# shuaigroup/Renormalizer

Hardware: AMD Instinct MI355X
Metric: TDVP-PS sweep site-updates/sec at (Nsite=50, Dbond=256, dphys=2/16) (higher is better)
Workload: dtype c128

## Files before the change

renormalizer_amd/csrc/mpse_gemm.hip:

```cpp
#include <cstdlib>

#include "mpse_device.h"
#include "mpse_internal.h"
#include "mpse_plans.h"

typedef double v4d __attribute__((ext_vector_type(4)));

static unsigned long long* gemm_trace_ptr(const mpse_ctx* ctx) {
  static const bool f0_only = [] {
    const char* e = getenv("MPSE_GEMM_TRACE_ONLY");
    return e && e[0] == 'f';
  }();
  return (ctx->prof_on && !f0_only) ? ctx->gemm_trace : nullptr;
}

namespace {

struct IdxMap {
  long long s_hi, s_lo;
  int ext, lo;
};

constexpr int GMAX_GRP = 8, GMAX_SEG = 4, GMAX_MIX = 8;
struct GMix {
  const double* src;
  int b, f, delta, pad;
};
struct GSeg {
  const double* A;
  const double* B;
  const unsigned char* am;
  const unsigned char* bm;
};
struct GGrp {
  GSeg seg[GMAX_SEG];
  double* C;
  int nseg;
  int use_beta;
};
struct GemmGroups {
  GGrp g[GMAX_GRP];
  int ngrp, tiles_m_grp, nkt_seg, am_pitch, bm_pitch;
  int split2, cpd;
  double* C2;
  const unsigned long long* flags;
  int nmix, mix_grp, mix_d, mix_wr;
  long long mix_ld;
  const double* mix_w;
  GMix mix[GMAX_MIX];
};

struct GemmArgs {
  const double* A;
  const double* B;
  double* C;
  IdxMap mA, kA, kB, nB, mC, nC;
  long long sbA, sbB, sbC;
  int M, N, K;
  int tiles_m, tiles_n;
  int mtiles_m, mtiles_n;
  int a_kfast, b_kfast;
  int conjA, conjB;
  int use_beta;
  double alpha_re, alpha_im, beta_re, beta_im;
  int skew;
  int die_group;
  int slice_fast;
  const int* perm;
  int ksplit;
  int kt_per_split;
  double* ws;
  const unsigned long long* amask;
  const unsigned long long* bmask;
  int nkw;
  unsigned long long* kt_counter;
  const int* skip;
  const double* dot_y;
  double* dot_part;
  const double* Cin;
  IdxMap mCin, nCin;
  unsigned long long* trace;
  GemmGroups gg;
};


__device__ __forceinline__ void dot_acc(double& re, double& im, double2 c, double2 y) {
  re += c.x * y.x + c.y * y.y;
  im += c.x * y.y - c.y * y.x;
}

__device__ __forceinline__ long long idx_off(const IdxMap& m, int i) {
  if (m.lo == 0x7fffffff) return (long long)i * m.s_lo;
  const int hi = i / m.lo;
  const int l = i - hi * m.lo;
  return (long long)hi * m.s_hi + (long long)l * m.s_lo;
}

#ifndef MPSE_GEMM_3M
#define MPSE_GEMM_3M 1
#endif
constexpr int BM = 64, BN = 64, BK = 16, LDK = BK + 1;

template <bool CA, bool CB, bool KS, int WS, int WI = 2, bool GRP = false>
__global__ __launch_bounds__(64 * WS * WS * (2 / WI), WS == 1 ? 1 : WI == 1 ? 4 : ((CA && CB) ? 2 : 3)) void k_gemm(const GemmArgs g) {
  static_assert(!GRP || (KS && WS == 2), "grouped launches use the single-level 64 x 64 kernel");
  constexpr int TBM = 32 * WS, TBN = 32 * WS, NT = 64 * WS * WS * (2 / WI);
  static_assert(WI == 2 || (WI == 1 && WS == 2), "eight-wave form only for 64 x 64 tiles");
  constexpr int LD = WS == 2 ? 80 : 48;
  constexpr int NLD = TBM * BK / NT;
  constexpr bool CC = CA || CB;
  constexpr int EA = CA ? 2 : 1, EB = CB ? 2 : 1, EC = CC ? 2 : 1;
  __shared__ double smem[(2 + (CA ? 1 : 0) + (CB ? 1 : 0)) * BK * LD];
  if (g.skip && *g.skip) return;
  const unsigned long long tr0 = g.trace ? __builtin_readcyclecounter() : 0ull;
  const unsigned long long rt0 = g.trace ? __builtin_amdgcn_s_memrealtime() : 0ull;
  unsigned long long tr1 = 0, tr2 = 0, tr3 = 0;
  double* sAr = smem;
  double* sAi = sAr + BK * LD;
  double* sBr = smem + (CA ? 2 : 1) * BK * LD;
  double* sBi = sBr + BK * LD;

  const int tid = threadIdx.x;
  const int lane = tid & 63;
  const int wave = tid >> 6;
  const int wm = WS == 2 ? wave >> 1 : 0, wn = WS == 2 ? wave & 1 : 0;
  constexpr int WROWS = 16 * WI;

  const int ntile = g.tiles_m * g.tiles_n;
  const int bid = blockIdx.x;
  int bs = bid / ntile;
  int t = bid - bs * ntile;
  int half = 0;
  if constexpr (GRP) {
    if (g.gg.split2) {
      if ((ntile & 7) == 0) {
        const int m2 = 2 * (ntile >> 3), r = bid >> 3, cpd = g.gg.cpd;
        const int q = (r < cpd || m2 <= cpd) ? r : (m2 - 1) - (r - cpd);
        half = q & 1;
        t = ((q >> 1) << 3) | (bid & 7);
      } else {
        half = bid & 1;
        t = bid >> 1;
      }
      bs = half;
    }
  }
  if (g.slice_fast) {
    t = bid / g.ksplit;
    bs = bid - t * g.ksplit;
  }
  const int b = bs / g.ksplit;
  const int ks_id = bs - b * g.ksplit;
  if (g.perm) t = g.perm[(ks_id & 1) ? ntile - 1 - t : t];
  int tm = t / g.tiles_n;
  int tn = t - tm * g.tiles_n;
  if (g.die_group == 1) {
    const int x = t & 7, j = t >> 3;
    tm = x + 8 * (j / g.tiles_n);
    tn = j % g.tiles_n;
  } else if (g.die_group == 2) {
    const int x = t & 7, j = t >> 3;
    tn = x + 8 * (j / g.tiles_m);
    tm = j % g.tiles_m;
  }
  if (g.skew && !g.perm && !g.die_group) tn = (tn + tm) % g.tiles_n;

  int grp = 0;
  if constexpr (GRP) {
    grp = tm / g.gg.tiles_m_grp;
    tm -= grp * g.gg.tiles_m_grp;
  }
  const GGrp& gp = g.gg.g[grp];
  const double* A = GRP ? gp.seg[0].A : g.A + (long long)b * g.sbA * EA;
  const double* B = GRP ? gp.seg[0].B : g.B + (long long)b * g.sbB * EB;
  double* C = GRP ? (half ? g.gg.C2 : gp.C) : g.C + (long long)b * g.sbC * EC;

  int ai[NLD], ak[NLD], bj[NLD], bk[NLD];
  long long aoff[NLD], boff[NLD];
#pragma unroll
  for (int r = 0; r < NLD; ++r) {
    if (g.a_kfast) {
      ak[r] = tid % BK;
      ai[r] = tid / BK + (NT / BK) * r;
    } else {
      ai[r] = tid % TBM;
      ak[r] = tid / TBM + (NT / TBM) * r;
    }
    if (g.b_kfast) {
      bk[r] = tid % BK;
      bj[r] = tid / BK + (NT / BK) * r;
    } else {
      bj[r] = tid % TBN;
      bk[r] = tid / TBN + (NT / TBN) * r;
    }
    int gi = min(tm * TBM + ai[r], g.M - 1);
    int gj = min(tn * TBN + bj[r], g.N - 1);
    aoff[r] = idx_off(g.mA, gi);
    boff[r] = idx_off(g.nB, gj);
  }

  double2 ra[NLD], rb[NLD];
  bool ka_in[NLD], kb_in[NLD];
  auto load_edge = [&](int kt) {
#pragma unroll
    for (int r = 0; r < NLD; ++r) {
      {
        const int k = kt * BK + ak[r];
        const bool kin = k < g.K;
        const int kc = kin ? k : g.K - 1;
        const long long ko = KS ? (long long)kc * g.kA.s_lo : idx_off(g.kA, kc);
        const double* p = A + (aoff[r] + ko) * EA;
        double2 v;
        if constexpr (CA) {
          v = *reinterpret_cast<const double2*>(p);
        } else {
          v.x = *p;
          v.y = 0.0;
        }
        ra[r] = v;
        ka_in[r] = kin;
      }
      {
        const int k = kt * BK + bk[r];
// ... 82 lines not shown
    const char* bt = b_col0 + (long long)kt * step_b;
    if constexpr (GRP) {
      const int q = kt / nkt_seg, l = kt - q * nkt_seg;
      at = seg_pick(seg_a, q) + (long long)l * step_a;
      bt = seg_pick(seg_b, q) + (long long)l * step_b;
    }
#pragma unroll
    for (int r = 0; r < NLD; ++r) {
      if constexpr (CA) {
        ra[r] = *reinterpret_cast<const double2*>(at + loa[r]);
      } else {
        ra[r].x = *reinterpret_cast<const double*>(at + loa[r]);
        ra[r].y = 0.0;
      }
      if constexpr (CB) {
        rb[r] = *reinterpret_cast<const double2*>(bt + lob[r]);
      } else {
        rb[r].x = *reinterpret_cast<const double*>(bt + lob[r]);
        rb[r].y = 0.0;
      }
    }
  };
  auto load_tile = [&](int kt) {
    if constexpr (GRP) {
      load_full(kt);
    } else if constexpr (KS) {
      if ((kt + 1) * BK <= g.K)
        load_full(kt);
      else
        load_ks(kt, false);
    } else {
      load_edge(kt);
    }
  };
  const double sgn_a = g.conjA ? -1.0 : 1.0, sgn_b = g.conjB ? -1.0 : 1.0;

  constexpr bool M3 = CA && CB && MPSE_GEMM_3M;
  v4d acc_re[WI][2], acc_im[WI][2], acc_t2[WI][2];
#pragma unroll
  for (int i = 0; i < WI; ++i)
#pragma unroll
    for (int j = 0; j < 2; ++j) {
      acc_re[i][j] = v4d{0, 0, 0, 0};
      acc_im[i][j] = v4d{0, 0, 0, 0};
      acc_t2[i][j] = v4d{0, 0, 0, 0};
    }

  constexpr int MASKW = 64;
  __shared__ unsigned long long s_mask[2][MASKW];
  const unsigned long long* am = nullptr;
  const unsigned long long* bm = nullptr;
  bool mlds = false;
  if constexpr (GRP) {
    if (g.nkw > 0 && g.nkw <= MASKW && g.gg.flags) {
      if (tid < g.nkw) {
        s_mask[0][tid] = g.gg.flags[((long long)(grp * g.gg.tiles_m_grp + tm) * g.tiles_n + tn) * g.nkw + tid];
        s_mask[1][tid] = 0x0101010101010101ull;
      }
      __syncthreads();
      mlds = true;
      am = s_mask[0];
    } else if (g.nkw > 0 && g.nkw <= MASKW) {
      unsigned char* f0 = reinterpret_cast<unsigned char*>(s_mask[0]);
      for (int t = tid; t < g.nkw * 8; t += NT) {
        unsigned char v = 0;
        if (t < nkt_all) {
          const int q = t / nkt_seg, l = t - q * nkt_seg;
          const GSeg& sg = gp.seg[q];
          v = 1;
          if (sg.am) v &= sg.am[(long long)tm * g.gg.am_pitch + l];
          if (sg.bm) v &= sg.bm[(long long)tn * g.gg.bm_pitch + l];
        }
        f0[t] = v;
      }
      if (tid < g.nkw) s_mask[1][tid] = 0x0101010101010101ull;
      __syncthreads();
      mlds = true;
      am = s_mask[0];
    }
    if (g.gg.split2) {
      if (mlds) {
        auto word_of = [&](int w) {
          unsigned long long x = s_mask[0][w] & 0x0101010101010101ull;
          const int valid = nkt_all - 8 * w;
          if (valid < 8) x &= valid > 0 ? (1ull << (8 * valid)) - 1ull : 0ull;
          return x;
        };
        int n = 0;
        for (int w = 0; w < g.nkw; ++w) n += __popcll(word_of(w));
        auto pos_of = [&](int i) {
          if (i >= n) return nkt_all;
          int seen = 0;
          for (int w = 0; w < g.nkw; ++w) {
            unsigned long long x = word_of(w);
            const int c = __popcll(x);
            if (seen + c > i) {
              for (int skip = i - seen; skip > 0; --skip) x &= x - 1;
              return (w << 3) + (__builtin_ctzll(x) >> 3);
            }
            seen += c;
          }
          return nkt_all;
        };
        kt_begin = half == 0 ? 0 : pos_of(n / 2);
        kt_end = half == 0 ? pos_of(n / 2) : nkt_all;
      } else {
        kt_begin = half == 0 ? 0 : nkt_all / 2;
        kt_end = half == 0 ? nkt_all / 2 : nkt_all;
      }
    }
  } else if constexpr (KS) {
    if (g.amask) am = g.amask + ((long long)b * g.mtiles_m + (tm * TBM) / BM) * g.nkw;
    if (g.bmask) bm = g.bmask + ((long long)b * g.mtiles_n + (tn * TBN) / BN) * g.nkw;
    if ((am || bm) && g.nkw <= MASKW) {
      if (tid < g.nkw) {
        s_mask[0][tid] = am ? am[tid] : 0x0101010101010101ull;
        s_mask[1][tid] = bm ? bm[tid] : 0x0101010101010101ull;
      }
      __syncthreads();
      mlds = true;
    }
  }
  auto next_kt = [&](int from) -> int {
    if (!am && !bm) return from;
    while (from < kt_end) {
      const int w = from >> 3;
      unsigned long long word = 0x0101010101010101ull;
      if (mlds) {
        word &= s_mask[0][w] & s_mask[1][w];
      } else {
        if (am) word &= am[w];
        if (bm) word &= bm[w];
      }
      word &= ~0ull << ((from & 7) * 8);
      if (word) {
        const int kt = (w << 3) + (__builtin_ctzll(word) >> 3);
        return kt < kt_end ? kt : kt_end;
      }
      from = (w + 1) << 3;
    }
    return kt_end;
  };
  int kt = next_kt(kt_begin);
  if (g.trace) tr1 = __builtin_readcyclecounter();
  if (kt < kt_end) {
    load_tile(kt);
  }
  const int frow = lane & 15, fk = lane >> 4;
  const int sai = g.a_kfast ? LDK : 1, sak = g.a_kfast ? 1 : LD;
  const int sbj = g.b_kfast ? LDK : 1, sbk = g.b_kfast ? 1 : LD;
  int wofa[NLD], wofb[NLD], rofa[WI], rofb[2];
#pragma unroll
  for (int r = 0; r < NLD; ++r) {
    wofa[r] = ai[r] * sai + ak[r] * sak;
    wofb[r] = bj[r] * sbj + bk[r] * sbk;
  }
#pragma unroll
  for (int i = 0; i < 2; ++i) {
// ... 362 lines not shown
        }
      }
    }
  }
  if constexpr (WS == 2) {
    if (g.dot_y) {
      __shared__ double s_dot[2 * (NT / 64)];
      dre = wave_sum(dre);
      dim = wave_sum(dim);
      if (lane == 0) {
        s_dot[2 * wave] = dre;
        s_dot[2 * wave + 1] = dim;
      }
      __syncthreads();
      dre = dim = 0.0;
#pragma unroll
      for (int w = 0; w < NT / 64; ++w) {
        dre += s_dot[2 * w];
        dim += s_dot[2 * w + 1];
      }
      if (tid == 0) {
        const long long slot = (long long)bs * ntile + (long long)tm * g.tiles_n + tn;
        g.dot_part[2 * slot] = dre;
        g.dot_part[2 * slot + 1] = dim;
      }
    }
  }
}

__device__ __forceinline__ void bitonic_desc(unsigned* key, int tid, int n) {
  for (int size = 2; size <= n; size <<= 1)
    for (int stride = size >> 1; stride > 0; stride >>= 1) {
      if (tid < (n >> 1)) {
        const int lo = 2 * tid - (tid & (stride - 1)), hi = lo + stride;
        const bool desc = (lo & size) == 0;
        const unsigned a = key[lo], b = key[hi];
        if ((a < b) == desc) {
          key[lo] = b;
          key[hi] = a;
        }
      }
      __syncthreads();
    }
}
__device__ __forceinline__ int pow2_at_least(int x) {
  int n = 2;
  while (n < x) n <<= 1;
  return n;
}
__global__ __launch_bounds__(1024) void k_tile_order(const unsigned long long* __restrict__ amask,
                                                       const unsigned long long* __restrict__ bmask, int nkw, int nkt,
                                                       int tiles_m, int tiles_n, int by_die, int* __restrict__ perm,
                                                       const int* __restrict__ skip, const GemmGroups gg,
                                                       unsigned char* __restrict__ flags_out, int flags_pitch) {
  if (skip && *skip) return;
  __shared__ unsigned key[2048], ckey[2048];
  __shared__ int colw[2048];
  __shared__ unsigned char die_of[2048];
  const int ntile = tiles_m * tiles_n, tid = threadIdx.x;
  const bool part = by_die && tiles_n % 8 == 0 && tiles_n <= 2048;
  for (int c = tid; c < 2048; c += 1024) colw[c] = 0;
  __syncthreads();
  for (int i = tid; i < 2048; i += 1024) {
    unsigned cnt = 0;
    if (i < ntile) {
      const int tm = i / tiles_n, tn = i - tm * tiles_n;
      if (gg.ngrp > 0) {
        const int grp = tm / gg.tiles_m_grp, tml = tm - grp * gg.tiles_m_grp;
        const GGrp& G = gg.g[grp];
        for (int q = 0; q < G.nseg; ++q)
          for (int l = 0; l < gg.nkt_seg; ++l) {
            unsigned v = 1;
            if (G.seg[q].am) v &= G.seg[q].am[(long long)tml * gg.am_pitch + l];
            if (G.seg[q].bm) v &= G.seg[q].bm[(long long)tn * gg.bm_pitch + l];
            cnt += v;
            if (flags_out) flags_out[(long long)i * flags_pitch + q * gg.nkt_seg + l] = (unsigned char)v;
          }
        if (flags_out)
          for (int l = G.nseg * gg.nkt_seg; l < flags_pitch; ++l) flags_out[(long long)i * flags_pitch + l] = 0;
      } else {
        for (int w = 0; w < nkw; ++w) {
          unsigned long long x = 0x0101010101010101ull;
          if (amask) x &= amask[(long long)tm * nkw + w];
          if (bmask) x &= bmask[(long long)tn * nkw + w];
          const int valid = nkt - 8 * w;
          if (valid < 8) x &= (1ull << (8 * valid)) - 1ull;
          cnt += __popcll(x);
        }
      }
      if (part) atomicAdd(&colw[tn], (int)cnt);
    }
    key[i] = cnt;
  }
  __syncthreads();
  if (part) {
    for (int c = tid; c < 2048; c += 1024) ckey[c] = c < tiles_n ? ((unsigned)colw[c] << 11) | (unsigned)(2047 - c) : 0u;
    __syncthreads();
    bitonic_desc(ckey, tid, pow2_at_least(tiles_n));
    for (int r = tid; r < tiles_n; r += 1024) {
      const int c = 2047 - (int)(ckey[r] & 2047u), r16 = r & 15;
      die_of[c] = (unsigned char)(r16 < 8 ? r16 : 15 - r16);
    }
    __syncthreads();
  }
  for (int i = tid; i < 2048; i += 1024) {
    unsigned k = 0;
    if (i < ntile) {
      const unsigned die = part ? die_of[i % tiles_n] : 0u;
      k = (die << 28) | (key[i] << 16) | (unsigned)(0xFFFF - i);
    }
    key[i] = k;
  }
  __syncthreads();
  bitonic_desc(key, tid, pow2_at_least(ntile));
  const int per_die = ntile / 8;
  for (int i = tid; i < ntile; i += 1024) {
    const int s = part ? (7 - (i & 7)) * per_die + (i >> 3) : i;
    perm[i] = 0xFFFF - (int)(key[s] & 0xFFFFu);
  }
}

template <bool CC>
__global__ __launch_bounds__(256) void k_splitk_reduce(const GemmArgs g, int batch) {
  constexpr int EC = CC ? 2 : 1;
  if (g.skip && *g.skip) return;
  const long long mn = (long long)g.M * g.N;
  const int rows = g.M * batch;
  double dre = 0.0, dim = 0.0;
  for (int row = blockIdx.y; row < rows; row += gridDim.y) {
    const int b = row / g.M;
    const int i = row - b * g.M;
    const double* wrow = g.ws + ((long long)b * g.ksplit * mn + (long long)i * g.N) * EC;
    double* crow = g.C + ((long long)b * g.sbC + idx_off(g.mC, i)) * EC;
    for (int j = blockIdx.x * 256 + threadIdx.x; j < g.N; j += gridDim.x * 256) {
      const double* w = wrow + (long long)j * EC;
      double xr = 0, xi = 0;
      int s = 0;
      for (; s + 4 <= g.ksplit; s += 4) {
        if constexpr (CC) {
          const double2 v0 = *reinterpret_cast<const double2*>(w + (long long)s * mn * EC);
          const double2 v1 = *reinterpret_cast<const double2*>(w + (long long)(s + 1) * mn * EC);
          const double2 v2 = *reinterpret_cast<const double2*>(w + (long long)(s + 2) * mn * EC);
          const double2 v3 = *reinterpret_cast<const double2*>(w + (long long)(s + 3) * mn * EC);
          xr += v0.x;
          xi += v0.y;
          xr += v1.x;
          xi += v1.y;
          xr += v2.x;
          xi += v2.y;
          xr += v3.x;
          xi += v3.y;
        } else {
          const double v0 = w[(long long)s * mn], v1 = w[(long long)(s + 1) * mn];
          const double v2 = w[(long long)(s + 2) * mn], v3 = w[(long long)(s + 3) * mn];
          xr += v0;
          xr += v1;
          xr += v2;
          xr += v3;
        }
      }
      for (; s < g.ksplit; ++s) {
        if constexpr (CC) {
          const double2 v = *reinterpret_cast<const double2*>(w + (long long)s * mn * EC);
          xr += v.x;
          xi += v.y;
        } else {
          xr += w[(long long)s * mn];
        }
      }
      const long long co = idx_off(g.nC, j);
      double* p = crow + co * EC;
// ... 332 lines not shown
  if (p.leave_slices) {
    g.ws = static_cast<double*>(rq->slices);
    rq->slices_used = g.ksplit;
  } else if (g.ksplit > 1) {
    MPSE_TRY(WSB.alloc(p.ws_bytes));
    g.ws = WSB.as<double>();
  }
  if (p.dot_producers) {
    g.dot_y = static_cast<const double*>(dot->y);
    g.dot_part = dot->part;
    dot->nb_out = (int)p.dot_producers;
  }
  mpse_ctx::ProfRec rec;
  const int variant = (ca ? 1 : 0) + (cb ? 2 : 0);
  const double mnk = double(g.M) * double(g.N) * double(g.K) * double(d->batch);
  const bool prof_this = prof_begin(
      ctx, variant, mnk * ((ca && cb) ? 8.0 : (ca || cb) ? 4.0 : 2.0),
      double(d->batch) * (double(g.M) * g.K * (ca ? 16 : 8) + double(g.K) * g.N * (cb ? 16 : 8) +
                          double(g.M) * g.N * ((ca || cb) ? 16 : 8) * (g.use_beta ? 2 : 1)),
      &rec);
  g.kt_counter = prof_this && ctx->prof_ktiles ? ctx->prof_ktiles + variant : nullptr;

  OccMask ma, mb;
  if (p.masks) {
    g.nkw = p.nkw;
    const bool sa = skip_zero & 1, sb = skip_zero & 2;
    const SolveScope::OccKey ka = occ_key(g.A, g.mA, g.kA, g.sbA, d->batch, ca);
    const SolveScope::OccKey kb = occ_key(g.B, g.nB, g.kB, g.sbB, d->batch, cb);
    SolveScope* const keep_a = sa && sc && sc->in_env(g.A) ? sc : nullptr;
    SolveScope* const keep_b = sb && sc && sc->in_env(g.B) ? sc : nullptr;
    const void* centre = (sb && sc && sc->in_krylov(g.B) && d->batch == 1 && (long long)occ_bytes(kb) == sc->cmask.bytes)
                             ? sc->cmask.ptr : nullptr;
    const size_t tmp_a = sa && !keep_a ? occ_bytes(ka) : 0, tmp_b = sb && !keep_b && !centre ? occ_bytes(kb) : 0;
    if (tmp_a + tmp_b) MPSE_TRY(MSK.alloc(tmp_a + tmp_b));
    if (sa) MPSE_TRY(occ_mask_source(ctx, keep_a, ka, nullptr, MSK.p, &ma));
    if (sb) MPSE_TRY(occ_mask_source(ctx, keep_b, kb, centre, MSK.as<char>() + tmp_a, &mb));
    if (ma.scan || mb.scan) {
      const OccOperand oa = occ_operand(ka, g.mA, g.kA, g.a_kfast, ma), ob = occ_operand(kb, g.nB, g.kB, g.b_kfast, mb);
      const dim3 og((p.nkt + 3) / 4, oa.tiles > ob.tiles ? oa.tiles : ob.tiles, (unsigned)(2 * d->batch));
      hipLaunchKernelGGL(k_tile_occ, og, dim3(256), 0, ctx->stream, oa, ob, g.K, g.nkw, (int)d->batch, g.skip);
    }
    g.amask = static_cast<const unsigned long long*>(ma.mask);
    g.bmask = static_cast<const unsigned long long*>(mb.mask);
  }

  if (p.order) {
    SolveScope* const keep = sc && sc->keeps_env_masks && ma.stable && mb.stable ? sc : nullptr;
    int* pp = nullptr;
    bool sort = false;
    MPSE_TRY(perm_source(ctx, keep, {g.amask, g.bmask, g.tiles_m, g.tiles_n, p.nkt, nullptr},
                         size_t(g.tiles_m) * g.tiles_n * sizeof(int), PERM, &pp, &sort));
    if (sort)
      hipLaunchKernelGGL(k_tile_order, dim3(1), dim3(1024), 0, ctx->stream, g.amask, g.bmask, g.nkw, p.nkt, g.tiles_m,
                         g.tiles_n, 1, pp, g.skip, GemmGroups(), (unsigned char*)nullptr, 0);
    g.perm = pp;
  }

  count_paths(ctx->gemm_paths, p, d->batch > 1);
  const bool reduce = g.ksplit > 1 && !p.leave_slices;
  launch_gemm(ctx, g, p.nwg, ca, cb, p.fast, p.wide, false, reduce ? dim3((unsigned)p.rgx, (unsigned)p.rgy) : dim3(0),
              (int)d->batch);
  if (prof_this) prof_end(ctx, rec);
  MPSE_HIP(ctx, hipGetLastError());
  return MPSE_OK;
}

int occ_mask_get(mpse_ctx* ctx, SolveScope* sc, const void* ptr, int dtype, mpse_index r, mpse_index k,
                 TmpBuf& tmp, const unsigned char** flags, int* pitch, bool* stable) {
  IdxMap rm, km;
  if (!to_map(r, &rm) || !to_map(k, &km) || !is_single(km))
    return mpse_fail(ctx, MPSE_ERR_SHAPE, "occupancy scan: K index must be single level");
  const SolveScope::OccKey key = occ_key(ptr, rm, km, 0, 1, dtype == MPSE_C128);
  SolveScope* const keep = sc && sc->in_env(ptr) ? sc : nullptr;
  OccMask m;
  if (!keep) MPSE_TRY(tmp.alloc(occ_bytes(key)));
  MPSE_TRY(occ_mask_source(ctx, keep, key, nullptr, tmp.p, &m));
  if (m.scan) {
    const OccOperand oa = occ_operand(key, rm, km, fastest(km) <= fastest(rm), m);
    OccOperand ob = oa;
    ob.tiles = 0;
    hipLaunchKernelGGL(k_tile_occ, dim3(((key.K + BK - 1) / BK + 3) / 4, key.tiles, 2), dim3(256), 0, ctx->stream, oa, ob,
                       key.K, key.nkw, 1, sc ? sc->skip : nullptr);
    MPSE_HIP(ctx, hipGetLastError());
  }
  *flags = static_cast<const unsigned char*>(m.mask);
  *pitch = key.nkw * 8;
  *stable = m.stable;
  return MPSE_OK;
}

static double mix_sources(const GroupedDesc& d) {
  int n = 0;
  for (int t = 0; t < d.nmix; ++t) {
    bool seen = false;
    for (int u = 0; u < t; ++u) seen = seen || d.mix[u].src == d.mix[t].src;
    n += seen ? 0 : 1;
  }
  return n > 1 ? double(n - 1) : 0.0;
}

int gemm_grouped(mpse_ctx* ctx, const GroupedDesc& d, SolveScope* sc, MatvecReq::Dot* dot) {
  GemmArgs g = {};
  if (d.ngrp < 1 || d.ngrp > GMAX_GRP) return mpse_fail(ctx, MPSE_ERR_ARG, "grouped product: 1 .. %d groups", GMAX_GRP);
  if (!fill_maps(g, d.ma, d.ka, d.kb, d.nb, d.mc, d.nc))
    return mpse_fail(ctx, MPSE_ERR_SHAPE, "grouped product: extent out of range");
  if (g.M != g.mC.ext || g.N != g.nC.ext || g.K != g.kB.ext) return mpse_fail(ctx, MPSE_ERR_SHAPE, "grouped product: extents disagree");
  if (g.M == 0 || g.N == 0) return MPSE_OK;
// ... 24 lines not shown
    gg.g[i].C = static_cast<double*>(s.C);
    gg.g[i].nseg = s.nseg;
    gg.g[i].use_beta = s.beta != 0.0 ? 1 : 0;
    if (s.beta != 0.0 && s.beta != 1.0) return mpse_fail(ctx, MPSE_ERR_ARG, "grouped product: beta must be 0 or 1");
    any_beta = any_beta || s.beta != 0.0;
    for (int q = 0; q < s.nseg; ++q) {
      if (!s.seg[q].A || !s.seg[q].B) return mpse_fail(ctx, MPSE_ERR_ARG, "grouped product: null operand");
      gg.g[i].seg[q] = GSeg{static_cast<const double*>(s.seg[q].A), static_cast<const double*>(s.seg[q].B), s.seg[q].am, s.seg[q].bm};
      any_mask = any_mask || s.seg[q].am || s.seg[q].bm;
    }
    max_seg = s.nseg > max_seg ? s.nseg : max_seg;
    segs += s.nseg;
  }
  g.A = gg.g[0].seg[0].A, g.B = gg.g[0].seg[0].B, g.C = gg.g[0].C;
  g.use_beta = any_beta;
  if (d.nmix > 0) {
    if (!ca || d.nmix > GMAX_MIX || d.mix_grp < 0 || d.mix_grp >= d.ngrp || d.grp[d.mix_grp].beta != 1.0 || !d.mix_w ||
        d.mix_d < 1 || BM % d.mix_d != 0 || g.M % BM != 0 || d.mix_wr < 1 || d.mix_ld < g.N)
      return mpse_fail(ctx, MPSE_ERR_ARG, "grouped product: bad epilogue mix");
    gg.nmix = d.nmix, gg.mix_grp = d.mix_grp, gg.mix_d = d.mix_d, gg.mix_wr = d.mix_wr, gg.mix_ld = d.mix_ld;
    gg.mix_w = static_cast<const double*>(d.mix_w);
    for (int t = 0; t < d.nmix; ++t) {
      if (!d.mix[t].src || d.mix[t].delta <= -d.mix_d || d.mix[t].delta >= d.mix_d)
        return mpse_fail(ctx, MPSE_ERR_ARG, "grouped product: bad epilogue mix term");
      gg.mix[t] = GMix{static_cast<const double*>(d.mix[t].src), d.mix[t].b, d.mix[t].f, d.mix[t].delta, 0};
    }
  }

  const int nkt_max = max_seg * gg.nkt_seg;
  const mpse_plan::GroupedPlan p = mpse_plan::grouped_plan(g.M, g.N, d.ngrp, nkt_max, any_mask, d.split2, ca, n_cu_of(ctx));
  const long long ntile = (long long)p.tiles_m * p.tiles_n;
  if (ntile > 0x7fffffffLL) return mpse_fail(ctx, MPSE_ERR_SHAPE, "grouped product: grid too large");
  g.tiles_m = p.tiles_m;
  g.nkw = p.nkw;
  g.die_group = p.die_group;
  if (dot && d.ngrp == 1 && p.nwg >= 1 && p.nwg <= dot->cap) {
    g.dot_y = static_cast<const double*>(dot->y);
    g.dot_part = dot->part;
    dot->nb_out = (int)p.nwg;
  }
  mpse_ctx::ProfRec rec;
  const int variant = (ca ? 1 : 0) + (cb ? 2 : 0);
  const double mnk = double(g.M) * double(g.N) * double(g.K) * segs;
  const bool prof_this = prof_begin(ctx, variant, mnk * ((ca && cb) ? 8.0 : 4.0),
                                    segs * (double(g.M) * g.K * (ca ? 16 : 8) + double(g.K) * g.N * 16.0) +
                                        double(d.ngrp) * double(g.M) * g.N * 16.0 * (any_beta ? 2 : 1) +
                                        mix_sources(d) * double(g.M) * g.N * 16.0,
                                    &rec);
  g.kt_counter = prof_this && ctx->prof_ktiles ? ctx->prof_ktiles + variant : nullptr;

  TmpBuf PERM(ctx);
  if (p.order) {
    const size_t perm_bytes = (size_t(ntile) * sizeof(int) + 7) & ~size_t(7), flag_pitch = size_t(g.nkw) * 8;
    int* pp = nullptr;
    bool sort = false;
    MPSE_TRY(perm_source(ctx, sc && sc->keeps_env_masks && d.masks_stable ? sc : nullptr,
                         {gg.g[0].seg[0].am, gg.g[0].seg[0].bm, g.tiles_m, g.tiles_n, nkt_max + 1000 * d.ngrp, nullptr},
                         perm_bytes + size_t(ntile) * flag_pitch, PERM, &pp, &sort));
    if (sort)
      hipLaunchKernelGGL(k_tile_order, dim3(1), dim3(1024), 0, ctx->stream, (const unsigned long long*)nullptr,
                         (const unsigned long long*)nullptr, 0, nkt_max, g.tiles_m, g.tiles_n, d.split2 ? 0 : 1, pp,
                         g.skip, gg, reinterpret_cast<unsigned char*>(pp) + perm_bytes, (int)flag_pitch);
    g.perm = pp;
    g.gg.flags = reinterpret_cast<const unsigned long long*>(reinterpret_cast<const char*>(pp) + perm_bytes);
  }

  count_paths(ctx->gemm_paths, d);
  launch_gemm(ctx, g, p.nwg, ca, cb, true, p.wide, true);
  if (prof_this) prof_end(ctx, rec);
  MPSE_HIP(ctx, hipGetLastError());
  return MPSE_OK;
}

extern "C" int mpse_gemm(mpse_ctx* ctx, const mpse_gemm_desc* d, const void* A, const void* B, void* C) {
  if (ctx && d && MPSE_RECORDING(ctx)) {
    const mpse_gemm_desc dc = *d;
    ctx->defer_ops[ctx->defer_recording].push_back([ctx, dc, A, B, C] { return mpse_gemm(ctx, &dc, A, B, C); });
    return MPSE_OK;
  }
  return gemm_impl(ctx, d, A, B, C, d ? (d->skip_zero_tiles & 3) : 0, nullptr, nullptr);
}

extern "C" int mpse_gemm_path_stats(mpse_ctx* ctx, int64_t* counts, int n) {
  if (!ctx || n < 0 || (n > 0 && !counts)) return MPSE_ERR_ARG;
  for (int i = 0; i < n && i < mpse_ctx::GP_COUNT; ++i) counts[i] = ctx->gemm_paths[i];
  return MPSE_OK;
}

int gemm_call(mpse_ctx* ctx, int dta, int dtb, int conja, int conjb, mpse_index ma, mpse_index ka, mpse_index kb,
              mpse_index nb, mpse_index mc, mpse_index nc, int64_t batch, int64_t sba, int64_t sbb, int64_t sbc,
              const void* A, const void* B, void* C, double alpha, double beta, int skip_zero, SolveScope* sc,
              ProductReq* rq) {
  mpse_gemm_desc d;
  d.dtype_a = dta;
  d.dtype_b = dtb;
  d.conj_a = conja;
  d.conj_b = conjb;
  d.m_a = ma;
  d.k_a = ka;
  d.k_b = kb;
  d.n_b = nb;
  d.m_c = mc;
  d.n_c = nc;
  d.batch = batch;
  d.sb_a = sba;
  d.sb_b = sbb;
  d.sb_c = sbc;
  d.alpha_re = alpha;
  d.alpha_im = 0.0;
  d.beta_re = beta;
  d.beta_im = 0.0;
  d.skip_zero_tiles = skip_zero;
  return gemm_impl(ctx, &d, A, B, C, skip_zero, sc, rq);
}

extern "C" int mpse_transpose_inner(mpse_ctx* ctx, int dtype, void* out, const void* in, int64_t d0, int64_t d1,
// ... 17 lines not shown
```

renormalizer_amd/csrc/mpse_internal.h:

```cpp
#pragma once
#include <hip/hip_runtime.h>

#include <cstdarg>
#include <cstdlib>
#include <cstdint>
#include <cstdio>
#include <cstring>
#include <functional>
#include <map>
#include <memory>
#include <mutex>
#include <string>
#include <unordered_map>
#include <vector>

#include "../../include/mpsengine.h"

struct mpse_ctx {
  int device = 0;
  hipStream_t stream = nullptr;
  int n_cu = 0;
  char err[512] = {0};
  char dev_name[128] = {0};

// ... 15 lines not shown
  std::vector<ProfRec> prof_pending;
  std::vector<hipEvent_t> prof_free_events;
  static constexpr int PROF_NVAR = 8;
  int64_t prof_svd_sweeps = 0;
  double prof_ms[PROF_NVAR] = {0};
  double prof_flops[PROF_NVAR] = {0};
  double prof_bytes[PROF_NVAR] = {0};
  int64_t prof_launches[PROF_NVAR] = {0};
  unsigned long long* prof_ktiles = nullptr;

  char* stage = nullptr;
  char* stage_dev = nullptr;
  size_t stage_size = 0, stage_pos = 0;

  enum PinnedSlot {
    PIN_SCALAR2 = 0,
    PIN_FLAG = 8,
    PIN_LZ_SCAL = 16,
    PIN_LZ_CTL = 24,
    PIN_ENV_UNIT = 32,
    PIN_PCG_CTL = 40,
    PIN_DAVIDSON = 64,
    PIN_BATCH_CTL = 3700,
    PIN_QR_STATUS = 3990,
    PIN_SLOTS_END = 4000,
    PIN_DOUBLES = 4096,
    PIN_SEQ = PIN_DOUBLES - 1
  };
  double* pinned = nullptr;
  double* pinned_dev = nullptr;
  unsigned long long publish_seq = 0;
  double* dscratch = nullptr;
  unsigned int flag_gen = 0;
  std::unordered_map<unsigned long long, int> lz_hint;
  struct WSiteEntry {
    std::shared_ptr<void> info;
    size_t bytes = 0;
  };
  std::unordered_map<const void*, WSiteEntry> wsite_info;
  std::vector<std::function<int()>> defer_ops[2];
  int defer_recording = -1;
  int defer_armed = -1;
  bool defer_hold = false;
  std::vector<void*> defer_frees;
  struct CMask {
    const void* ptr = nullptr;
    long long bytes = 0;
  } cmask_pending;
  unsigned long long* gemm_trace = nullptr;
  bool gemm_trace_checked = false;
  long long f0_launches[2] = {0, 0};
  enum GemmPath {
    GP_LAUNCH, GP_GENERAL, GP_WIDE, GP_SPLIT_B1, GP_SPLIT_BN, GP_DIE1, GP_DIE2, GP_SKEW, GP_ORDER, GP_MASK,
    GP_MASK_GLOBAL, GP_GROUPED, GP_GROUPED_SPLIT2, GP_GROUPED_MIX, GP_WMIX, GP_COUNT
  };
  long long gemm_paths[GP_COUNT] = {0};
  long long qr_chol_calls = 0, qr_chol_fallbacks = 0, qr_calls = 0;
  bool qr_optimistic = false;
  int qr_scheme = -1;
  int* qr_words_dev = nullptr;
  long long lz_batch_members = 0, lz_batch_single = 0;
  enum LzPath {
    LP_SYNC, LP_ASYNC_DONE, LP_HOST_FIRST, LP_HOST_LATER, LP_LIMIT, LP_BD_ASYNC, LP_BD_SYNC, LP_FULL, LP_CONV,
    LP_NOCONV, LP_MERGED, LP_WAITS, LP_GROW, LP_PARTS, LP_VMASK, LP_UNVEC, LP_RESCALE, LP_ALIAS_RESTART, LP_COUNT
  };
  long long lz_paths[LP_COUNT] = {0};
  enum PcgStat {
    PS_SOLVES, PS_ITERS, PS_MATVECS, PS_WAITS, PS_END_TOL, PS_END_MAXITER, PS_END_CURVATURE, PS_TWOLAYER, PS_MASKED,
    PS_COUNT
  };
  long long pcg_stats[PS_COUNT] = {0};
  enum PcgSumStat { PSS_SOLVES, PSS_ITERS, PSS_TERM_APPLIES, PSS_WAITS, PSS_DIAGS, PSS_COUNT };
  long long pcg_sum_stats[PSS_COUNT] = {0};
  enum PcgBatchStat { PB_MEMBERS, PB_SINGLE, PB_SETS, PB_MATVEC_LAUNCHES, PB_WAITS, PB_COUNT };
  long long pcg_batch_stats[PB_COUNT] = {0};
  enum OverlapStat { OV_CHAIN, OV_ENQUEUED, OV_SITES, OV_COUNT };
  long long overlap_stats[OV_COUNT] = {0};
  enum SandwichStat { SW_CHAIN, SW_ENQUEUED, SW_SITES, SW_COUNT };
  long long sandwich_stats[SW_COUNT] = {0};
  enum CorrStat { CR_CHAIN, CR_ENQUEUED, CR_SITES, CR_ENTRIES, CR_COUNT };
  long long corr_stats[CR_COUNT] = {0};
};
int qr_words(mpse_ctx* ctx);

int mpse_fail(mpse_ctx* ctx, int code, const char* fmt, ...);
inline int mpse_bind(mpse_ctx* ctx) {
  int cur = -1;
  if (hipGetDevice(&cur) == hipSuccess && cur == ctx->device) return MPSE_OK;
  if (hipSetDevice(ctx->device) != hipSuccess) return mpse_fail(ctx, MPSE_ERR_HIP, "hipSetDevice(%d) failed", ctx->device);
  return MPSE_OK;
}
int stage_h2d(mpse_ctx* ctx, void* dst, const void* src_host, size_t bytes);
int device_zero(mpse_ctx* ctx, void* dst, size_t bytes);
inline void wsite_written(mpse_ctx* ctx, const void* dst, size_t bytes) {
  if (!dst || !bytes) return;
  std::lock_guard<std::mutex> lock(ctx->pool_mu);
  if (ctx->wsite_info.empty()) return;
  const char* lo = static_cast<const char*>(dst);
  for (auto it = ctx->wsite_info.begin(); it != ctx->wsite_info.end();) {
    const char* w = static_cast<const char*>(it->first);
    if (lo < w + it->second.bytes && w < lo + bytes)
      it = ctx->wsite_info.erase(it);
    else
      ++it;
  }
}
void prof_drain(mpse_ctx* ctx);
// ... 294 lines not shown
```

renormalizer_amd/engine.py:

```python
import collections
import ctypes as C
import math
import os
import threading

import numpy as np

_HERE = os.path.dirname(os.path.abspath(__file__))
LIB_PATH = os.environ.get("RENO_MPSENGINE") or os.path.join(_HERE, "csrc", "libmpsengine.so")

F64, C128 = 0, 1
MPSE_OK, MPSE_ERR_OOM, MPSE_ERR_SHAPE, MPSE_ERR_NOCONV, MPSE_ERR_HIP, MPSE_ERR_ARG = 0, 1, 2, 3, 4, 5
DOMAIN_L, DOMAIN_R = 0, 1

STATUS = {0: "OK", 1: "OOM", 2: "SHAPE", 3: "NOCONV", 4: "HIP", 5: "ARG"}


PcgResult = collections.namedtuple("PcgResult", "status iters relres lvalue")


class EngineError(RuntimeError):
    pass


# ... 664 lines not shown
    @staticmethod
    def corr_dims(sites):
        rows = []
        for i, t in enumerate(sites):
            if t.ndim not in (3, 4):
                raise ValueError(f"mps_corr: site {i} has shape {t.shape}")
            rows.append([t.shape[0], t.shape[1], t.shape[2] if t.ndim == 4 else 1, t.shape[-1]])
        return rows

    def mps_corr(self, sites, sel, x_mats, y_mats, z_mats):
        rows = self.corr_dims(sites)
        n, nsel = len(rows), len(sel)
        if n == 0 or nsel == 0 or not (len(x_mats) == len(y_mats) == len(z_mats) == nsel):
            raise ValueError(f"mps_corr: {n} sites, {nsel} selected, {len(x_mats)}/{len(y_mats)}/{len(z_mats)} matrices")
        packed = []
        for mats in (x_mats, y_mats, z_mats):
            flat = []
            for k, m in zip(sel, mats):
                m = np.ascontiguousarray(m, dtype=np.complex128)
                d = rows[k][1] if 0 <= int(k) < n else m.shape[0]
                if m.shape != (d, d):
                    raise ValueError(f"mps_corr: a local matrix of site {k} has shape {m.shape}, the site has d = {d}")
                flat.append(m.reshape(-1))
            packed.append(np.ascontiguousarray(np.concatenate(flat)).view(np.float64))
        dims = (C.c_int64 * (4 * n))(*[int(x) for r in rows for x in r])
        out = np.zeros((nsel, nsel), dtype=np.complex128)
        self._check(self.lib.mpse_mps_corr(
            self.ctx, n, *_site_args(sites), dims, nsel, (C.c_int * nsel)(*[int(k) for k in sel]),
            *[p.ctypes.data_as(_dblp) for p in packed], out.ctypes.data_as(_dblp)))
        return out

    def block_qr_stats(self):
        a, b, c = C.c_int64(), C.c_int64(), C.c_int64()
        self._check(self.lib.mpse_block_qr_stats(self.ctx, C.byref(a), C.byref(b), C.byref(c)))
        return a.value, b.value, c.value

    def heff_fused_stats(self):
        a, b = C.c_int64(), C.c_int64()
        self._check(self.lib.mpse_heff_fused_stats(self.ctx, C.byref(a), C.byref(b)))
        return a.value, b.value

    GEMM_PATHS = ("launches", "general", "eight_wave", "split_b1", "split_batched", "die_group1", "die_group2", "skew",
                  "tile_order", "masks", "masks_global", "grouped", "grouped_split2")

    def gemm_path_stats(self):
        return self._stats_dict(self.lib.mpse_gemm_path_stats, self.GEMM_PATHS)

    def wfold_path_stats(self):
        n = len(self.GEMM_PATHS)
        v = (C.c_int64 * (n + 2))()
        self._check(self.lib.mpse_gemm_path_stats(self.ctx, v, n + 2))
        return {"grouped_mix": int(v[n]), "wmix": int(v[n + 1])}

    def block_qr_optimistic(self, on):
        self._check(self.lib.mpse_block_qr_optimistic(self.ctx, int(bool(on))))

    def block_qr_scheme(self, scheme):
        self._check(self.lib.mpse_block_qr_scheme(self.ctx, int(scheme)))

    def block_qr_check(self):
        v = C.c_int(0)
        self._check(self.lib.mpse_block_qr_check(self.ctx, C.byref(v)))
        return bool(v.value)

    def block_qr_pass_stats(self):
        a, b = C.c_int64(0), C.c_int64(0)
        self._check(self.lib.mpse_block_qr_pass_stats(self.ctx, C.byref(a), C.byref(b)))
        return a.value, b.value

    def prof_get(self):
        names = {0: "f64xf64", 1: "c128xf64", 2: "f64xc128", 3: "c128xc128", 4: "lanczos_vec", 5: "block_qr", 6: "block_svd",
                 7: "heff_fused"}
        issued_per_mac = {0: 2.0, 1: 4.0, 2: 4.0, 3: 6.0}
        out = {}
        for v, nm in names.items():
            ms, fl, by, n = C.c_double(), C.c_double(), C.c_double(), C.c_int64()
            self._check(self.lib.mpse_prof_get(self.ctx, v, C.byref(ms), C.byref(fl), C.byref(by), C.byref(n)))
            out[nm] = dict(ms=ms.value, flops=fl.value, bytes=by.value, launches=n.value)
            if v < 4:
                kt = C.c_int64()
                self._check(self.lib.mpse_prof_get_ktiles(self.ctx, v, C.byref(kt)))
                out[nm]["ktiles"] = kt.value
                out[nm]["issued_flops"] = kt.value * 65536.0 * issued_per_mac[v]
        sw = C.c_int64()
        self._check(self.lib.mpse_prof_get_svd_sweeps(self.ctx, C.byref(sw)))
        out["block_svd"]["sweeps"] = sw.value
        return out

    def empty(self, shape, dtype=np.float64):
        if isinstance(shape, (int, np.integer)):
            shape = (shape,)
        dtype = np.dtype(dtype)
        dtype_code(dtype)
        n = math.prod(int(x) for x in shape)
        buf = _Buffer(self, n * dtype.itemsize)
        return DeviceTensor(self, buf, 0, shape, dtype)

    def zeros(self, shape, dtype=np.float64):
        t = self.empty(shape, dtype)
        self._check(self.lib.mpse_memset_zero(self.ctx, t.ptr, t.nbytes))
        return t

    def asdevice(self, a, dtype=None):
        if isinstance(a, DeviceTensor):
            if dtype is not None and np.dtype(dtype) != a.dtype:
                if np.dtype(dtype) == np.complex128:
# ... 80 lines not shown
```

Before: 600.9.

## Precompute per-workgroup tile records for grouped GEMM in tile-order kernel

The tile-order kernel now writes one compact record per workgroup. Each record holds the group, tile coordinates, split half, k-range and occupancy bits. The grouped GEMM kernel reads its record instead of recomputing the split2 position, reading the permutation, gathering the per-tile flag words and doing the popcount-based half-range search at kernel start. This is meant to shorten the prologue of every grouped GEMM workgroup and drop a __syncthreads, at the cost of extra work and memory in the single-block tile-order kernel. It is limited to nkw <= 8 and can be turned off with an environment variable.

```diff
diff --git a/renormalizer_amd/csrc/mpse_gemm.hip b/renormalizer_amd/csrc/mpse_gemm.hip
--- a/renormalizer_amd/csrc/mpse_gemm.hip
+++ b/renormalizer_amd/csrc/mpse_gemm.hip
@@ -1,6 +1,7 @@
 #include <cstdlib>
 
 #include "mpse_device.h"
+#include "mpse_gemm_rec.h"
 #include "mpse_internal.h"
 #include "mpse_plans.h"
 
@@ -44,6 +45,7 @@
   int split2, cpd;
   double* C2;
   const unsigned long long* flags;
+  const GemmRec* recs;
   int nmix, mix_grp, mix_d, mix_wr;
   long long mix_ld;
   const double* mix_w;
@@ -111,6 +113,20 @@
   constexpr bool CC = CA || CB;
   constexpr int EA = CA ? 2 : 1, EB = CB ? 2 : 1, EC = CC ? 2 : 1;
   __shared__ double smem[(2 + (CA ? 1 : 0) + (CB ? 1 : 0)) * BK * LD];
+  bool has_rec = false;
+  int rec_grp = 0, rec_tm = 0, rec_tn = 0, rec_half = 0, rec_kb = 0, rec_ke = 0;
+  unsigned long long rec_word = 0ull;
+  if constexpr (GRP) {
+    if (g.gg.recs) {
+      const GemmRec* rp = g.gg.recs + blockIdx.x;
+      has_rec = true;
+      rec_grp = __builtin_amdgcn_readfirstlane(rp->grp), rec_tm = __builtin_amdgcn_readfirstlane(rp->tm);
+      rec_tn = __builtin_amdgcn_readfirstlane(rp->tn), rec_half = __builtin_amdgcn_readfirstlane(rp->half);
+      rec_kb = __builtin_amdgcn_readfirstlane(rp->kt_begin), rec_ke = __builtin_amdgcn_readfirstlane(rp->kt_end);
+      rec_word = grec_word(rp->bits, threadIdx.x & (GREC_W - 1));
+      asm volatile("" ::: "memory");
+    }
+  }
   if (g.skip && *g.skip) return;
   const unsigned long long tr0 = g.trace ? __builtin_readcyclecounter() : 0ull;
   const unsigned long long rt0 = g.trace ? __builtin_amdgcn_s_memrealtime() : 0ull;
@@ -132,16 +148,11 @@
   int t = bid - bs * ntile;
   int half = 0;
   if constexpr (GRP) {
-    if (g.gg.split2) {
-      if ((ntile & 7) == 0) {
-        const int m2 = 2 * (ntile >> 3), r = bid >> 3, cpd = g.gg.cpd;
-        const int q = (r < cpd || m2 <= cpd) ? r : (m2 - 1) - (r - cpd);
-        half = q & 1;
-        t = ((q >> 1) << 3) | (bid & 7);
-      } else {
-        half = bid & 1;
-        t = bid >> 1;
-      }
+    if (has_rec) {
+      half = rec_half;
+      if (g.gg.split2) bs = half;
+    } else if (g.gg.split2) {
+      grec_split2_pos(bid, ntile, g.gg.cpd, &t, &half);
       bs = half;
     }
   }
@@ -151,7 +162,7 @@
   }
   const int b = bs / g.ksplit;
   const int ks_id = bs - b * g.ksplit;
-  if (g.perm) t = g.perm[(ks_id & 1) ? ntile - 1 - t : t];
+  if (g.perm && !(GRP && has_rec)) t = g.perm[(ks_id & 1) ? ntile - 1 - t : t];
   int tm = t / g.tiles_n;
   int tn = t - tm * g.tiles_n;
   if (g.die_group == 1) {
@@ -167,8 +178,12 @@
 
   int grp = 0;
   if constexpr (GRP) {
-    grp = tm / g.gg.tiles_m_grp;
-    tm -= grp * g.gg.tiles_m_grp;
+    if (has_rec) {
+      grp = rec_grp, tm = rec_tm, tn = rec_tn;
+    } else {
+      grp = tm / g.gg.tiles_m_grp;
+      tm -= grp * g.gg.tiles_m_grp;
+    }
   }
   const GGrp& gp = g.gg.g[grp];
   const double* A = GRP ? gp.seg[0].A : g.A + (long long)b * g.sbA * EA;
@@ -357,7 +372,16 @@
   const unsigned long long* bm = nullptr;
   bool mlds = false;
   if constexpr (GRP) {
-    if (g.nkw > 0 && g.nkw <= MASKW && g.gg.flags) {
+    if (has_rec) {
+      if (lane < GREC_W) {
+        s_mask[0][lane] = rec_word;
+        s_mask[1][lane] = 0x0101010101010101ull;
+      }
+      mlds = true;
+      am = s_mask[0];
+      kt_begin = rec_kb;
+      kt_end = rec_ke;
+    } else if (g.nkw > 0 && g.nkw <= MASKW && g.gg.flags) {
       if (tid < g.nkw) {
         s_mask[0][tid] = g.gg.flags[((long long)(grp * g.gg.tiles_m_grp + tm) * g.tiles_n + tn) * g.nkw + tid];
         s_mask[1][tid] = 0x0101010101010101ull;
@@ -383,32 +407,9 @@
       mlds = true;
       am = s_mask[0];
     }
-    if (g.gg.split2) {
+    if (g.gg.split2 && !has_rec) {
       if (mlds) {
-        auto word_of = [&](int w) {
-          unsigned long long x = s_mask[0][w] & 0x0101010101010101ull;
-          const int valid = nkt_all - 8 * w;
-          if (valid < 8) x &= valid > 0 ? (1ull << (8 * valid)) - 1ull : 0ull;
-          return x;
-        };
-        int n = 0;
-        for (int w = 0; w < g.nkw; ++w) n += __popcll(word_of(w));
-        auto pos_of = [&](int i) {
-          if (i >= n) return nkt_all;
-          int seen = 0;
-          for (int w = 0; w < g.nkw; ++w) {
-            unsigned long long x = word_of(w);
-            const int c = __popcll(x);
-            if (seen + c > i) {
-              for (int skip = i - seen; skip > 0; --skip) x &= x - 1;
-              return (w << 3) + (__builtin_ctzll(x) >> 3);
-            }
-            seen += c;
-          }
-          return nkt_all;
-        };
-        kt_begin = half == 0 ? 0 : pos_of(n / 2);
-        kt_end = half == 0 ? pos_of(n / 2) : nkt_all;
+        grec_half_range([&](int w) { return s_mask[0][w]; }, g.nkw, nkt_all, half, &kt_begin, &kt_end);
       } else {
         kt_begin = half == 0 ? 0 : nkt_all / 2;
         kt_end = half == 0 ? nkt_all / 2 : nkt_all;
@@ -877,17 +878,24 @@
                                                        const unsigned long long* __restrict__ bmask, int nkw, int nkt,
                                                        int tiles_m, int tiles_n, int by_die, int* __restrict__ perm,
                                                        const int* __restrict__ skip, const GemmGroups gg,
-                                                       unsigned char* __restrict__ flags_out, int flags_pitch) {
+                                                       unsigned char* __restrict__ flags_out, int flags_pitch,
+                                                       GemmRec* __restrict__ recs) {
   if (skip && *skip) return;
   __shared__ unsigned key[2048], ckey[2048];
   __shared__ int colw[2048];
   __shared__ unsigned char die_of[2048];
+  __shared__ unsigned long long tbits[2048];
+  __shared__ int s_nseg[GMAX_GRP];
+#pragma unroll
+  for (int q = 0; q < GMAX_GRP; ++q)
+    if ((int)threadIdx.x == q) s_nseg[q] = gg.g[q].nseg;
   const int ntile = tiles_m * tiles_n, tid = threadIdx.x;
   const bool part = by_die && tiles_n % 8 == 0 && tiles_n <= 2048;
   for (int c = tid; c < 2048; c += 1024) colw[c] = 0;
   __syncthreads();
   for (int i = tid; i < 2048; i += 1024) {
     unsigned cnt = 0;
+    unsigned long long bits = 0ull;
     if (i < ntile) {
       const int tm = i / tiles_n, tn = i - tm * tiles_n;
       if (gg.ngrp > 0) {
@@ -899,6 +907,7 @@
             if (G.seg[q].am) v &= G.seg[q].am[(long long)tml * gg.am_pitch + l];
             if (G.seg[q].bm) v &= G.seg[q].bm[(long long)tn * gg.bm_pitch + l];
             cnt += v;
+            bits |= (unsigned long long)v << ((q * gg.nkt_seg + l) & 63);
             if (flags_out) flags_out[(long long)i * flags_pitch + q * gg.nkt_seg + l] = (unsigned char)v;
           }
         if (flags_out)
@@ -916,6 +925,7 @@
       if (part) atomicAdd(&colw[tn], (int)cnt);
     }
     key[i] = cnt;
+    tbits[i] = bits;
   }
   __syncthreads();
   if (part) {
@@ -942,6 +952,24 @@
   for (int i = tid; i < ntile; i += 1024) {
     const int s = part ? (7 - (i & 7)) * per_die + (i >> 3) : i;
     perm[i] = 0xFFFF - (int)(key[s] & 0xFFFFu);
+  }
+  if (recs) {
+    const int nwg = gg.split2 ? 2 * ntile : ntile;
+    for (int pos = tid; pos < nwg; pos += 1024) {
+      int tpos = pos, half = 0;
+      if (gg.split2) grec_split2_pos(pos, ntile, gg.cpd, &tpos, &half);
+      const int s = part ? (7 - (tpos & 7)) * per_die + (tpos >> 3) : tpos;
+      const int t = 0xFFFF - (int)(key[s] & 0xFFFFu);
+      const int tmg = t / tiles_n;
+      GemmRec r;
+      r.grp = tmg / gg.tiles_m_grp, r.tm = tmg - r.grp * gg.tiles_m_grp, r.tn = t - tmg * tiles_n;
+      r.half = half, r.pad = 0;
+      r.bits = tbits[t], r.pad2 = 0ull;
+      const int nkt_all = s_nseg[r.grp] * gg.nkt_seg;
+      r.kt_begin = 0, r.kt_end = nkt_all, r.nocc = __popcll(r.bits);
+      if (gg.split2) grec_half_range_bits(r.bits, nkt_all, half, &r.kt_begin, &r.kt_end);
+      recs[pos] = r;
+    }
   }
 }
 
@@ -1380,7 +1408,7 @@
                          size_t(g.tiles_m) * g.tiles_n * sizeof(int), PERM, &pp, &sort));
     if (sort)
       hipLaunchKernelGGL(k_tile_order, dim3(1), dim3(1024), 0, ctx->stream, g.amask, g.bmask, g.nkw, p.nkt, g.tiles_m,
-                         g.tiles_n, 1, pp, g.skip, GemmGroups(), (unsigned char*)nullptr, 0);
+                         g.tiles_n, 1, pp, g.skip, GemmGroups(), (unsigned char*)nullptr, 0, (GemmRec*)nullptr);
     g.perm = pp;
   }
 
@@ -1511,16 +1539,25 @@
   TmpBuf PERM(ctx);
   if (p.order) {
     const size_t perm_bytes = (size_t(ntile) * sizeof(int) + 7) & ~size_t(7), flag_pitch = size_t(g.nkw) * 8;
+    static const bool records_on = [] {
+      const char* e = getenv("MPSE_GEMM_RECORDS");
+      return !(e && e[0] == '0');
+    }();
+    const bool records = records_on && g.nkw <= GREC_W;
+    const size_t rec_off = (perm_bytes + size_t(ntile) * flag_pitch + 15) & ~size_t(15);
     int* pp = nullptr;
     bool sort = false;
     MPSE_TRY(perm_source(ctx, sc && sc->keeps_env_masks && d.masks_stable ? sc : nullptr,
                          {gg.g[0].seg[0].am, gg.g[0].seg[0].bm, g.tiles_m, g.tiles_n, nkt_max + 1000 * d.ngrp, nullptr},
-                         perm_bytes + size_t(ntile) * flag_pitch, PERM, &pp, &sort));
+                         rec_off + (records ? size_t(p.nwg) * sizeof(GemmRec) : 0), PERM, &pp, &sort));
+    GemmRec* const recs = records ? reinterpret_cast<GemmRec*>(reinterpret_cast<char*>(pp) + rec_off) : nullptr;
     if (sort)
       hipLaunchKernelGGL(k_tile_order, dim3(1), dim3(1024), 0, ctx->stream, (const unsigned long long*)nullptr,
                          (const unsigned long long*)nullptr, 0, nkt_max, g.tiles_m, g.tiles_n, d.split2 ? 0 : 1, pp,
-                         g.skip, gg, reinterpret_cast<unsigned char*>(pp) + perm_bytes, (int)flag_pitch);
+                         g.skip, gg, reinterpret_cast<unsigned char*>(pp) + perm_bytes, (int)flag_pitch, recs);
     g.perm = pp;
+    g.gg.recs = recs;
+    ctx->gemm_paths[mpse_ctx::GP_GROUPED_REC] += records;
     g.gg.flags = reinterpret_cast<const unsigned long long*>(reinterpret_cast<const char*>(pp) + perm_bytes);
   }
 
diff --git a/renormalizer_amd/csrc/mpse_gemm_rec.h b/renormalizer_amd/csrc/mpse_gemm_rec.h
--- /dev/null
+++ b/renormalizer_amd/csrc/mpse_gemm_rec.h
@@ -0,0 +1,82 @@
+#pragma once
+
+#if defined(__HIPCC__) || defined(__CUDACC__)
+#define MPSE_REC_HD __host__ __device__ __forceinline__
+#else
+#define MPSE_REC_HD inline
+#endif
+
+constexpr int GREC_W = 8;
+
+struct alignas(16) GemmRec {
+  int grp, tm, tn;
+  int half;
+  int kt_begin, kt_end;
+  int nocc;
+  int pad;
+  unsigned long long bits, pad2;
+};
+
+MPSE_REC_HD unsigned long long grec_word(unsigned long long bits, int w) {
+  const unsigned b8 = (unsigned)(bits >> (8 * w)) & 0xFFu;
+  const unsigned lo = ((b8 & 0xFu) * 0x00204081u) & 0x01010101u, hi = ((b8 >> 4) * 0x00204081u) & 0x01010101u;
+  return ((unsigned long long)hi << 32) | lo;
+}
+
+MPSE_REC_HD void grec_split2_pos(int pos, int ntile, int cpd, int* tpos, int* half) {
+  if ((ntile & 7) == 0) {
+    const int m2 = 2 * (ntile >> 3), r = pos >> 3;
+    const int q = (r < cpd || m2 <= cpd) ? r : (m2 - 1) - (r - cpd);
+    *half = q & 1;
+    *tpos = ((q >> 1) << 3) | (pos & 7);
+  } else {
+    *half = pos & 1;
+    *tpos = pos >> 1;
+  }
+}
+
+template <class Word>
+MPSE_REC_HD int grec_half_range(Word word, int nkw, int nkt_all, int half, int* kt_begin, int* kt_end) {
+  auto word_of = [&](int w) {
+    unsigned long long x = word(w) & 0x0101010101010101ull;
+    const int valid = nkt_all - 8 * w;
+    if (valid < 8) x &= valid > 0 ? (1ull << (8 * valid)) - 1ull : 0ull;
+    return x;
+  };
+  int n = 0;
+  for (int w = 0; w < nkw; ++w) n += __builtin_popcountll(word_of(w));
+  int mid = nkt_all;
+  if (n / 2 < n) {
+    int seen = 0;
+    for (int w = 0; w < nkw; ++w) {
+      unsigned long long x = word_of(w);
+      const int c = __builtin_popcountll(x);
+      if (seen + c > n / 2) {
+        for (int skip = n / 2 - seen; skip > 0; --skip) x &= x - 1;
+        mid = (w << 3) + (__builtin_ctzll(x) >> 3);
+        break;
+      }
+      seen += c;
+    }
+  }
+  *kt_begin = half == 0 ? 0 : mid;
+  *kt_end = half == 0 ? mid : nkt_all;
+  return n;
+}
+
+MPSE_REC_HD int grec_half_range_bits(unsigned long long bits, int nkt_all, int half, int* kt_begin, int* kt_end) {
+  if (nkt_all < 64) bits &= nkt_all > 0 ? (1ull << nkt_all) - 1ull : 0ull;
+  const int n = __builtin_popcountll(bits);
+  int mid = nkt_all;
+  if (n > 0) {
+    int k = n / 2, pos = 0;
+    for (int width = 32; width > 0; width >>= 1) {
+      const int c = __builtin_popcountll((bits >> pos) & ((1ull << width) - 1ull));
+      if (k >= c) pos += width, k -= c;
+    }
+    mid = pos;
+  }
+  *kt_begin = half == 0 ? 0 : mid;
+  *kt_end = half == 0 ? mid : nkt_all;
+  return n;
+}
diff --git a/renormalizer_amd/csrc/mpse_internal.h b/renormalizer_amd/csrc/mpse_internal.h
--- a/renormalizer_amd/csrc/mpse_internal.h
+++ b/renormalizer_amd/csrc/mpse_internal.h
@@ -91,7 +91,7 @@
   long long f0_launches[2] = {0, 0};
   enum GemmPath {
     GP_LAUNCH, GP_GENERAL, GP_WIDE, GP_SPLIT_B1, GP_SPLIT_BN, GP_DIE1, GP_DIE2, GP_SKEW, GP_ORDER, GP_MASK,
-    GP_MASK_GLOBAL, GP_GROUPED, GP_GROUPED_SPLIT2, GP_GROUPED_MIX, GP_WMIX, GP_COUNT
+    GP_MASK_GLOBAL, GP_GROUPED, GP_GROUPED_SPLIT2, GP_GROUPED_MIX, GP_WMIX, GP_GROUPED_REC, GP_COUNT
   };
   long long gemm_paths[GP_COUNT] = {0};
   long long qr_chol_calls = 0, qr_chol_fallbacks = 0, qr_calls = 0;
diff --git a/renormalizer_amd/engine.py b/renormalizer_amd/engine.py
--- a/renormalizer_amd/engine.py
+++ b/renormalizer_amd/engine.py
@@ -740,6 +740,12 @@
         self._check(self.lib.mpse_gemm_path_stats(self.ctx, v, n + 2))
         return {"grouped_mix": int(v[n]), "wmix": int(v[n + 1])}
 
+    def gemm_record_stats(self):
+        n = len(self.GEMM_PATHS) + 3
+        v = (C.c_int64 * n)()
+        self._check(self.lib.mpse_gemm_path_stats(self.ctx, v, n))
+        return int(v[n - 1])
+
     def block_qr_optimistic(self, on):
         self._check(self.lib.mpse_block_qr_optimistic(self.ctx, int(bool(on))))
 
```

Result: no change. 601.5 (median of 4 runs) (+0.1%).
